# Sweethyh/GaussianImage_plus

Hardware: AMD Instinct MI355X
Metric: training iters/sec (fwd+bwd rasterize) at N Gaussians, 768x512 (higher is better)
Workload: dtype f32; 1 GPU; Cholesky model, N=50000 Gaussians, 768x512, one image per GPU, whole training iterations with the optimizer ON (moving gaussians): tanh/+bound + project fwd + incremental tile binning + rasterize_sum fwd + L2 gradient of the render + rasterize_sum bwd + project bwd + Adam per step; num_points=50000, height=512, width=768, seed=3047

## Files before the change

gaussianimage_plus_amd/csrc/gi2d_common.h:

```cpp
#pragma once
#include <hip/hip_runtime.h>
#include <stdint.h>

#include "gi2d.h"

#define GI2D_WAVE 64
#define GI2D_BLOCK 256

namespace gi2d {

void set_error(const char *msg);
int check_launch(const char *what);

__device__ __forceinline__ int cvt_rzi(float x) {
    if (x != x) return 0;
    x = fminf(fmaxf(x, -2147483648.f), 2147483520.f);
    return (int)x;
}

__device__ __forceinline__ void tile_bbox(float cx, float cy, float pix_radius, int tiles_x,
                                          int tiles_y, int &min_x, int &min_y, int &max_x,
                                          int &max_y) {
#pragma clang fp contract(off)
    const float tcx = cx / (float)GI2D_TILE, tcy = cy / (float)GI2D_TILE;
// ... 55 lines not shown

struct ConicS {
    float ha, hb, hc;
};
__device__ __forceinline__ ConicS scale_conic(float a, float b, float c) {
    const float l2e = 1.4426950408889634f;
    ConicS s;
    s.ha = 0.5f * a * l2e;
    s.hb = b * l2e;
    s.hc = 0.5f * c * l2e;
    return s;
}
__device__ __forceinline__ float row_term_b(const ConicS &s, float dy) { return s.hb * dy; }
__device__ __forceinline__ float row_term_c(const ConicS &s, float dy) { return __builtin_fmaf(s.hc * dy, dy, 0.f); }
__device__ __forceinline__ float pair_sigma(const ConicS &s, float dx, float bdy, float cdy2) {
    return __builtin_fmaf(dx, __builtin_fmaf(s.ha, dx, bdy), cdy2);
}
__device__ __forceinline__ float pair_vis(float sigma_l2) { return __builtin_amdgcn_exp2f(-sigma_l2); }

struct AlphaRule {
    unsigned lim;
    bool clamp;
};
#define GI2D_LIM_ODD 0xffffffffu
__device__ __forceinline__ AlphaRule alpha_rule(float gx, float gy, float a, float b, float c, float opac) {
    AlphaRule r;
    const float s = gx + gy + a + b + c + opac;
    const bool odd = !(__builtin_fabsf(s) <= 3.4028235e38f);
    r.clamp = odd || !(opac <= 1.f);
    const float smax = __builtin_amdgcn_logf(opac * 255.f);
    r.lim = odd ? GI2D_LIM_ODD : (smax >= 0.f ? (unsigned)__float_as_int(smax) + 1u : 0u);
    return r;
}
__device__ __forceinline__ bool pair_lands(float sigma_l2, unsigned lim) { return (unsigned)__float_as_int(sigma_l2) < lim; }
__device__ __forceinline__ bool pair_lands_odd(float sigma_l2, float alpha_unclamped, unsigned lim) {
    unsigned as_written = (!(sigma_l2 < 0.f) & !(fminf(1.f, alpha_unclamped) < (1.f / 255.f))) ? 1u : 0u;
    unsigned fast = pair_lands(sigma_l2, lim) ? 1u : 0u;
    asm volatile("" : "+v"(as_written), "+v"(fast));
    return (lim == GI2D_LIM_ODD ? as_written : fast) != 0u;
}

struct CullBox {
    float x0, x1, y0, y1;
};
#define GI2D_CULL_FULL 3.0e38f
#ifndef GI2D_CULL_MARGIN
#define GI2D_CULL_MARGIN 0.0625f
#endif
__device__ __forceinline__ void cull_extent(float gx, float gy, float a, float b, float c, float opac, float &hx,
                                            float &hy) {
    const float big = GI2D_CULL_FULL;
    hx = hy = big;
    if (!(opac == opac)) return;
    if (!(opac * 255.f >= 1.f)) {
        hx = hy = -1.f;
        return;
    }
    const float det = a * c - b * b;
    if (!(a > 0.f) || !(c > 0.f) || !(det > 0.f)) return;
    const float tau2 = 2.f * __logf(opac * 255.f) * 1.0002f + 1e-3f;
    const float t = tau2 * __builtin_amdgcn_rcpf(det);
    const float ex = __builtin_amdgcn_sqrtf(t * c) * 1.0002f + GI2D_CULL_MARGIN;
    const float ey = __builtin_amdgcn_sqrtf(t * a) * 1.0002f + GI2D_CULL_MARGIN;
    if (!(ex < big) || !(ey < big) || !(gx == gx) || !(gy == gy)) return;
    hx = ex;
    hy = ey;
// ... 24 lines not shown
```

gaussianimage_plus_amd/csrc/gi2d_fast.hip:

```cpp
#include <cstdio>
#include <cstdlib>
#include <cstring>
#include <mutex>
#include <unordered_map>
#include <vector>

#include <hip/hip_ext.h>

#include "gi2d_fused_core.h"
#include "gi2d_batch.h"

namespace gi2d {

__global__ __launch_bounds__(256) void fast_fill_kernel(int n, const float2 *__restrict__ xys,
                                                        const int32_t *__restrict__ radii,
                                                        const float *__restrict__ conics,
                                                        const float *__restrict__ colors,
                                                        const float *__restrict__ opacities, int tiles_x, int tiles_y,
                                                        float radius_clip, PrevBox *__restrict__ prev_box,
                                                        int32_t *__restrict__ lists, RecSets rs,
                                                        int32_t *__restrict__ status) {
    const int g = blockIdx.x * blockDim.x + threadIdx.x;
    begin_binning(g, status);
    const BinRecs recs = recs_for_binning(rs, g == 0);
// ... 25 lines not shown
}

template <int KIND>
__global__ __launch_bounds__(256) void fast_project_fill_kernel(
    int n, float clip_coe, const float2 *__restrict__ means2d, const float *__restrict__ p0,
    const float *__restrict__ p1, float img_w, float img_h, int tiles_x, int tiles_y, float radius_clip,
    float2 *__restrict__ xys, float *__restrict__ depths, int32_t *__restrict__ radii,
    float *__restrict__ conics, int32_t *__restrict__ num_tiles_hit, BinTarget bt) {
    project_fill_one<KIND>(blockIdx.x * blockDim.x + threadIdx.x, n, clip_coe, means2d, p0, p1, img_w, img_h, tiles_x,
                           tiles_y, radius_clip, xys, depths, radii, conics, num_tiles_hit, bt);
}

struct FastFwdLds {
    FwdLds f;
};
static_assert(sizeof(float4) * GI2D_FWD_PAIRBUF >= sizeof(int) * GI2D_FAST_C, "the id buffer of the list head overlays the pair buffers");

template <bool WT>
__global__ __launch_bounds__(256) void fast_fwd_kernel(
    int tiles_x, int tiles_y, int img_w, int img_h, RecSets rs, const float *__restrict__ background,
    int32_t *__restrict__ lists, int2 *__restrict__ tile_bins,
    GaussRec *__restrict__ packed, float4 *__restrict__ partial_g, float4 *__restrict__ partial_big,
    int32_t *__restrict__ status, float *__restrict__ final_Ts, int32_t *__restrict__ final_idx,
    float *__restrict__ out_img) {
    __shared__ FastFwdLds sm;
    __shared__ int grp[32];
    int *ids = reinterpret_cast<int *>(sm.f.pairbuf);
    const int tile = blockIdx.x;
    const int tx = tile % tiles_x, ty = tile / tiles_x;
    const int tid = threadIdx.x;
    const float4 *recs = recs_for_tile_pass(rs, blockIdx.x == 0 && tid == 0);
    if (tid == 0) fwd_stage_dummy(sm.f);
    const float tx0 = (float)(tx * GI2D_TILE), ty0 = (float)(ty * GI2D_TILE);
    const int L = tile_list_head<false>(
        ids, grp, tile, tx, ty, recs, lists, tile_bins, status, [&](int, const BinRec &br) { return br; },
        [&](int rank, int g, const BinRec &br) {
            const GaussRec &r = br.r;
            int slot = partial_slot(g, br.box, tx, ty, br.pool);
            float4 *row = partial_row(slot, partial_g, partial_big, tiles_x * tiles_y * GI2D_TILE_LIST_CAP, status);
            if (!row) slot = GI2D_NO_ROW;
            if (rank < GI2D_TILE_LIST_CAP) {
                const AlphaRule ar = alpha_rule(r.gx, r.gy, r.a, r.b, r.c, r.opac);
                const unsigned mask = cull_word_ext(r.gx, r.gy, br.hx, br.hy, tx0, ty0, img_h, ar.clamp);
                fwd_stage_entry(sm.f, rank, r, mask, ar.lim);
                float4 *dst = reinterpret_cast<float4 *>(packed + (size_t)tile * GI2D_TILE_LIST_CAP + rank);
                store16<WT>(dst, make_float4(r.gx, r.gy, r.a, r.b), packed);
                store16<WT>(dst + 1, make_float4(r.c, r.opac, r.cr, r.cg), packed);
                store16<WT>(dst + 2, make_float4(r.cb, __int_as_float(slot), __int_as_float(g), __int_as_float((int)mask)), packed);
            } else if (row) {
                const float4 z = make_float4(0.f, 0.f, 0.f, 0.f);
                row[0] = z;
                row[1] = z;
                row[2] = z;
            }
        }, Inbox{nullptr}, head_row_load(lists, tile, false));
    __syncthreads();
    const int len = L > GI2D_TILE_LIST_CAP ? GI2D_TILE_LIST_CAP : L;
    const bool nothing = background != nullptr && !tile_pass_has_members(rs);
    if (final_idx)
        fwd_rasterize_staged<true, WT>(sm.f, len, list_base(tile), tx, ty, img_w, img_h, nothing, background,
                                       final_Ts, final_idx, out_img);
    else
        fwd_rasterize_staged<false, WT>(sm.f, len, list_base(tile), tx, ty, img_w, img_h, nothing, background,
                                        final_Ts, final_idx, out_img);
    if (tid == 0 && L > 0) status[0] = 1;
}

__global__ __launch_bounds__(256) void fast_background_kernel(int img_w, int img_h,
                                                              const int32_t *__restrict__ status,
                                                              const float *__restrict__ background,
                                                              float *__restrict__ out_img) {
    if (status[0] > 0) return;
    const size_t npix = (size_t)img_w * img_h;
    for (size_t p = blockIdx.x * (size_t)blockDim.x + threadIdx.x; p < npix; p += (size_t)gridDim.x * blockDim.x) {
        out_img[3 * p] = background[0];
        out_img[3 * p + 1] = background[1];
        out_img[3 * p + 2] = background[2];
    }
}

template <bool WITH_ABS, bool WT>
// ... 224 lines not shown
    BinTarget bt;
    int32_t *tile_order;
};

template <int KIND, bool FILL_NEXT>
__global__ __launch_bounds__(256) void fast_reduce_project_kernel(
    int n, int role_blocks, float2 *xys, int32_t *radii, float *conics, int tiles_x, int tiles_y, float radius_clip,
    PrevBox *prev_box, const int32_t *__restrict__ gids_sorted, const int2 *__restrict__ tile_bins,
    const float4 *__restrict__ partial_g, const float4 *__restrict__ partial_big, const float *__restrict__ p0,
    const float *__restrict__ p1, float img_w, float img_h, float2 *__restrict__ v_xy, float *__restrict__ v_conic,
    float *__restrict__ v_rgb, float *__restrict__ v_opacity, float4 *__restrict__ v_abs_xy,
    float *__restrict__ v_cov2d, float2 *__restrict__ v_mean2d, float *__restrict__ v_p0, float *__restrict__ v_p1,
    NextProject next) {
    int block = blockIdx.x;
    if (FILL_NEXT) {
        if (block >= 2 * role_blocks) {
            compute_tile_order(tile_bins, tiles_x * tiles_y, next.tile_order);
            return;
        }
        if (block >= role_blocks) {
            project_fill_one<KIND>((block - role_blocks) * blockDim.x + threadIdx.x, n, next.clip_coe, next.means2d, p0,
                                   p1, img_w, img_h, tiles_x, tiles_y, radius_clip, xys, next.depths, radii, conics,
                                   next.num_tiles_hit, next.bt);
            return;
        }
    }
    const int g = block * blockDim.x + threadIdx.x;
    int2 box = make_int2(0, 0);
    int pool = -1;
    float conic[3] = {0.f, 0.f, 0.f};
    int radius = 0;
    if (g < n) {
        if (FILL_NEXT) {
            const float4 *rec = recs_of_last_pass(next.bt.recs) + 4 * (size_t)g;
            const float4 q0 = rec[0], q1 = rec[1], q2 = rec[2], q3 = rec[3];
            conic[0] = q0.z, conic[1] = q0.w, conic[2] = q1.x;
            box = make_int2(__float_as_int(q2.w), __float_as_int(q3.x));
            radius = __float_as_int(q3.y);
            pool = __float_as_int(q3.z);
        } else {
            const PrevBox pb = prev_box[g];
            box = make_int2(pb.x, pb.y), pool = pb.z;
            conic[0] = conics[3 * g], conic[1] = conics[3 * g + 1], conic[2] = conics[3 * g + 2];
            radius = radii[g];
        }
    }
    float par[3] = {0.f, 0.f, 0.f};
    if (g < n) {
        if (KIND == kScaleRot)
            par[0] = p0[2 * g], par[1] = p0[2 * g + 1], par[2] = p1[g];
        else if (KIND == kCholesky)
            par[0] = p0[3 * g], par[1] = p0[3 * g + 1], par[2] = p0[3 * g + 2];
    }
    float acc[11];
    reduce_one(g, box, pool, tiles_x * tiles_y * GI2D_TILE_LIST_CAP, partial_g, partial_big, acc);
    if (g >= n) return;
    store_grads(g, acc, v_xy, v_conic, v_rgb, v_opacity, v_abs_xy);
    ProjGrad r;
    r.g11 = r.g12 = r.g22 = r.o0 = r.o1 = r.o2 = 0.f;
    r.v_mean = make_float2(0.f, 0.f);
    if (radius > 0) {
        const float vc[3] = {acc[2], acc[3], acc[4]};
        r = project_bwd_one<KIND>(0, par, par + 2, img_w, img_h, conic, make_float2(acc[0], acc[1]), vc);
    }
    store_proj_grad(g, KIND == kScaleRot, r, v_cov2d, v_mean2d, v_p0, v_p1);
}

static int check_ws(const char *what, void *ws, size_t ws_bytes, int n, int tiles_x, int tiles_y) {
    if (n < 0 || tiles_x < 0 || tiles_y < 0) {
        set_error("fast path: negative size");
        return GI2D_ERR_INVALID_ARGUMENT;
// ... 644 lines not shown
```

gaussianimage_plus_amd/csrc/gi2d_fast_internal.h:

```cpp
#pragma once
#include <atomic>
#include <type_traits>

#include "gi2d_project_core.h"
#include "gi2d_raster_core.h"

namespace gi2d {


#define GI2D_FAST_C 1024
#define GI2D_FAST_HDR 16
#define GI2D_INBOX_WORDS 64
#define GI2D_INBOX_SLOTS (32 * GI2D_INBOX_WORDS)
#define GI2D_INBOX_MAX_TILES 1536
#define GI2D_FAST_LROW (GI2D_FAST_C + GI2D_FAST_HDR + GI2D_INBOX_WORDS)
#define GI2D_FAST_EPT (GI2D_FAST_C / 256)
#define GI2D_FAST_S 32
#ifndef GI2D_FILL_BATCH
#define GI2D_FILL_BATCH 16
#endif
#ifndef GI2D_REDUCE_BATCH
#define GI2D_REDUCE_BATCH 8
#endif
#define GI2D_BIG_TILES_F 32
// ... 58 lines not shown
    GaussRec *packed;
    PrevBox *prev_box;
    float4 *recs;
    int32_t *ver;
    float4 *partial_g;
    float4 *partial_big;
    int32_t *tile_order;
    int32_t *big_tile;
    size_t bytes;
};
static FastWs carve_fast(void *base, int n, int num_tiles) {
    FastWs w;
    char *b = (char *)base;
    size_t off = 0;
    const size_t t = (size_t)(num_tiles > 0 ? num_tiles : 1), nn = (size_t)(n > 0 ? n : 1);
    w.inbox_recs = nullptr;
    w.lists = (int32_t *)(b + off);
    w.gids_sorted = w.lists;
    off += align_up(t * GI2D_FAST_LROW * sizeof(int32_t));
    w.tile_bins = (int32_t *)(b + off);
    off += align_up(t * 2 * sizeof(int32_t));
    w.packed = (GaussRec *)(b + off);
    off += align_up(t * GI2D_TILE_LIST_CAP * sizeof(GaussRec));
    w.tile_order = (int32_t *)(b + off);
    off += align_up(t * sizeof(int32_t));
    w.big_tile = (int32_t *)(b + off);
    off += align_up(t * sizeof(int32_t));
    w.prev_box = (PrevBox *)(b + off);
    off += align_up(nn * sizeof(PrevBox));
    w.ver = (int32_t *)(b + off);
    off += align_up(64 * sizeof(int32_t));
    w.recs = (float4 *)(b + off);
    off += 2 * align_up(nn * 4 * sizeof(float4));
    w.partial_g = (float4 *)(b + off);
    off += align_up(nn * GI2D_FAST_S * GI2D_FAST_ROW * sizeof(float4));
    w.partial_big = (float4 *)(b + off);
    off += align_up(t * GI2D_TILE_LIST_CAP * GI2D_FAST_ROW * sizeof(float4));
    w.bytes = off;
    return w;
}
static inline bool wt_fits(const FastWs &w, int num_tiles, size_t image_bytes) {
    const size_t rows_span = (size_t)((const char *)w.partial_big - (const char *)w.partial_g) +
                             (size_t)(num_tiles > 0 ? num_tiles : 1) * GI2D_TILE_LIST_CAP * GI2D_FAST_ROW * sizeof(float4);
    const size_t packed_span = (size_t)(num_tiles > 0 ? num_tiles : 1) * GI2D_TILE_LIST_CAP * sizeof(GaussRec);
    return rows_span < 0xffff0000ull && packed_span < 0xffff0000ull && image_bytes < 0xffff0000ull;
}
static inline size_t inbox_bytes(long long num_tiles) {
    if (num_tiles < 1 || num_tiles > GI2D_INBOX_MAX_TILES) return 0;
    return align_up((size_t)num_tiles * GI2D_INBOX_SLOTS * 4 * sizeof(float4));
}
__host__ __device__ __forceinline__ int list_base(int tile) { return tile * GI2D_FAST_LROW + GI2D_FAST_HDR; }

__device__ __forceinline__ int2 pack_box(int mnx, int mny, int mxx, int mxy) {
    return make_int2(mnx | (mxx << 16), mny | (mxy << 16));
}
struct FillPending {
    int c[GI2D_FILL_BATCH], p[GI2D_FILL_BATCH];
    int nt, w, mnx, mny, omnx, omxx, omny, omxy, di, dj;
    int pool;
    bool live;
};
#ifdef GI2D_INBOX_STATS
#define GI2D_INBOX_STAT(word) atomicAdd(&lists[word], 1)
#else
#define GI2D_INBOX_STAT(word) \
    do {                      \
// ... 120 lines not shown
template <bool INBOX = false>
__device__ __forceinline__ void fill_diff_end(int g, FillPending &f, int tiles_x, int32_t *__restrict__ lists,
                                              const InboxFill *in = nullptr) {
    if (f.nt == 0) return;
    fill_trip_store(f, g, lists);
    for (int base = GI2D_FILL_BATCH; base < f.nt; base += GI2D_FILL_BATCH) {
        fill_trip_issue<INBOX>(f, base, tiles_x, lists, in);
        fill_trip_store(f, g, lists);
    }
}
__device__ __forceinline__ void fill_diff(int g, bool member, int mnx, int mny, int mxx, int mxy, int tiles_x,
                                          PrevBox old, PrevBox *__restrict__ prev_box, int32_t *__restrict__ lists) {
    FillPending f = fill_diff_begin(g, member, mnx, mny, mxx, mxy, tiles_x, old, prev_box, lists);
    fill_diff_end(g, f, tiles_x, lists);
}
__device__ __forceinline__ bool bin_box(const float2 xy, int rad, float radius_clip, int tiles_x, int tiles_y, int &mnx,
                                        int &mny, int &mxx, int &mxy) {
    mnx = mny = mxx = mxy = 0;
    if (rad <= 0 || (float)rad < radius_clip) return false;
    tile_bbox(xy.x, xy.y, (float)rad, tiles_x, tiles_y, mnx, mny, mxx, mxy);
    return mxx > mnx && mxy > mny;
}
__device__ __forceinline__ bool tile_member(const float2 xy, int rad, float radius_clip, int tiles_x, int tiles_y,
                                            int tx, int ty, int &mnx, int &mny, int &mxx, int &mxy) {
    return bin_box(xy, rad, radius_clip, tiles_x, tiles_y, mnx, mny, mxx, mxy) && tx >= mnx && tx < mxx && ty >= mny &&
           ty < mxy;
}
struct RecSets {
    float4 *base;
    int32_t *ver;
    unsigned stride;
    int seq;
};
#define GI2D_VER_ANY 2
#define GI2D_VER_ANY_SEQ 3
#define GI2D_VER_LATEST 4
#define GI2D_VER_WORDS 5
static_assert(GI2D_VER_WORDS <= 16, "the stamps share the version words' 64 bytes; word 16 onwards has other owners");
struct BinRecs {
    float4 *recs;
    int32_t *any;
    int stamp, seq;
};
__device__ __forceinline__ BinRecs recs_for_binning(const RecSets &rs, bool writer) {
    const int c = rs.ver[0];
    BinRecs b;
    b.recs = rs.base + (size_t)((c + 1) & 1) * rs.stride;
    b.any = rs.ver + GI2D_VER_ANY;
    b.stamp = c + 1;
    b.seq = rs.seq;
    if (writer) rs.ver[1] = c + 1, rs.ver[GI2D_VER_LATEST] = rs.seq;
    return b;
}
__device__ __forceinline__ void note_member(const BinRecs &b) { b.any[0] = b.stamp, b.any[GI2D_VER_ANY_SEQ - GI2D_VER_ANY] = b.seq; }
__device__ __forceinline__ bool tile_pass_has_members(const RecSets &rs) {
    return rs.ver[GI2D_VER_ANY] == rs.ver[1] && rs.ver[GI2D_VER_ANY_SEQ] == rs.ver[GI2D_VER_LATEST];
}
__device__ __forceinline__ const float4 *recs_for_tile_pass(const RecSets &rs, bool writer) {
    const int b = rs.ver[1];
    if (writer) rs.ver[0] = b;
    return rs.base + (size_t)(b & 1) * rs.stride;
}
__device__ __forceinline__ const float4 *recs_of_last_pass(const RecSets &rs) {
    return rs.base + (size_t)(rs.ver[0] & 1) * rs.stride;
}
inline std::atomic<unsigned> g_call_seq{1};
static inline RecSets rec_sets(const FastWs &w, int n) {
    RecSets rs;
    rs.seq = (int)(g_call_seq.fetch_add(1, std::memory_order_relaxed) & 0x7fffffffu);
    rs.base = w.recs;
    rs.stride = (unsigned)(align_up((size_t)(n > 0 ? n : 1) * 4 * sizeof(float4)) / sizeof(float4));
    rs.ver = w.ver;
    return rs;
}
struct BinTarget {
    const float *colors, *opacities;
    PrevBox *prev_box;
    int32_t *lists;
    RecSets recs;
    int32_t *status;
};

__device__ __forceinline__ void begin_binning(int g, int32_t *__restrict__ status) {
    if (g == 0) {
        status[0] = 0;
        status[1] = 0;
        status[3] = 0;
    }
}
__device__ __forceinline__ void make_record(float4 (&q)[4], int g, float2 xy, float a, float b, float c, float opac,
                                            float cr, float cg, float cb, int2 box, int radius, int pool) {
    float hx, hy;
    cull_extent(xy.x, xy.y, a, b, c, opac, hx, hy);
    q[0] = make_float4(xy.x, xy.y, a, b);
    q[1] = make_float4(c, opac, cr, cg);
    q[2] = make_float4(cb, hx, hy, __int_as_float(box.x));
    q[3] = make_float4(__int_as_float(box.y), __int_as_float(radius), __int_as_float(pool), __int_as_float(g));
}
__device__ __forceinline__ void store_record(float4 *__restrict__ recs, int g, const float4 (&q)[4]) {
    float4 *r = recs + 4 * (size_t)g;
    r[0] = q[0], r[1] = q[1], r[2] = q[2], r[3] = q[3];
}
__device__ __forceinline__ void write_record(float4 *__restrict__ recs, int g, float2 xy, float a, float b, float c,
                                             float opac, float cr, float cg, float cb, int2 box, int radius, int pool) {
    float4 q[4];
    make_record(q, g, xy, a, b, c, opac, cr, cg, cb, box, radius, pool);
    store_record(recs, g, q);
}
struct BinRec {
    GaussRec r;
    float hx, hy;
    int2 box;
    int pool;
};
__device__ __forceinline__ BinRec record_of(const float4 q0, const float4 q1, const float4 q2, const float4 q3, int g) {
    BinRec o;
    o.r.gx = q0.x, o.r.gy = q0.y, o.r.a = q0.z, o.r.b = q0.w;
    o.r.c = q1.x, o.r.opac = q1.y, o.r.cr = q1.z, o.r.cg = q1.w;
    o.r.cb = q2.x, o.r.slot = -1, o.r.gid = g, o.r.pad = 0;
    o.hx = q2.y, o.hy = q2.z;
    o.box = make_int2(__float_as_int(q2.w), __float_as_int(q3.x));
    o.pool = __float_as_int(q3.z);
    return o;
}
__device__ __forceinline__ BinRec load_record(const float4 *__restrict__ recs, int g) {
    const float4 *p = recs + 4 * (size_t)g;
    const float4 q0 = p[0], q1 = p[1], q2 = p[2];
    const float4 q3 = p[3];
    return record_of(q0, q1, q2, q3, g);
}
__device__ __forceinline__ BinRec load_inbox_record(const float4 *__restrict__ p) {
    const float4 q0 = p[0], q1 = p[1], q2 = p[2];
    const float4 q3 = p[3];
    return record_of(q0, q1, q2, q3, __float_as_int(q3.w));
}
__device__ __forceinline__ void unpack_box(int2 box, int &mnx, int &mny, int &mxx, int &mxy) {
    mnx = box.x & 0xffff, mxx = (int)((unsigned)box.x >> 16), mny = box.y & 0xffff, mxy = (int)((unsigned)box.y >> 16);
}
template <bool INBOX = false, class Between>
__device__ __forceinline__ void bin_one(int g, float2 xy, int radius, bool has_tiles, float ka, float kb, float kc,
                                        float opac, float cr, float cg, float cb, int tiles_x, int tiles_y,
                                        float radius_clip, PrevBox old_box, PrevBox *__restrict__ prev_box,
                                        int32_t *__restrict__ lists, const BinRecs &br, Between between,
                                        InboxFill *in = nullptr) {
    int mnx, mny, mxx, mxy;
    const bool member = bin_box(xy, radius, radius_clip, tiles_x, tiles_y, mnx, mny, mxx, mxy) && has_tiles;
    {
        const unsigned long long mm = __ballot(member);
        if (mm != 0ull && (int)(threadIdx.x & 63) == __builtin_ctzll(mm)) note_member(br);
    }
    float4 *recs = br.recs;
    const int2 box = member ? pack_box(mnx, mny, mxx, mxy) : make_int2(0, 0);
    if constexpr (INBOX) {
        make_record(in->q, g, xy, ka, kb, kc, opac, cr, cg, cb, box, radius, old_box.z);
        FillPending f = fill_diff_begin<true>(g, member, mnx, mny, mxx, mxy, tiles_x, old_box, prev_box, lists, in);
        in->q[3].z = __int_as_float(f.pool);
        store_record(recs, g, in->q);
        between();
        fill_diff_end<true>(g, f, tiles_x, lists, in);
    } else {
        FillPending f = fill_diff_begin(g, member, mnx, mny, mxx, mxy, tiles_x, old_box, prev_box, lists);
        write_record(recs, g, xy, ka, kb, kc, opac, cr, cg, cb, box, radius, f.pool);
        between();
        fill_diff_end(g, f, tiles_x, lists);
    }
}
__device__ __forceinline__ void bin_one(int g, float2 xy, int radius, bool has_tiles, float ka, float kb, float kc,
                                        float opac, float cr, float cg, float cb, int tiles_x, int tiles_y,
                                        float radius_clip, PrevBox old_box, PrevBox *__restrict__ prev_box,
                                        int32_t *__restrict__ lists, const BinRecs &recs) {
    bin_one(g, xy, radius, has_tiles, ka, kb, kc, opac, cr, cg, cb, tiles_x, tiles_y, radius_clip, old_box, prev_box, lists,
            recs, [] {});
}
template <bool INBOX = false, class Between>
__device__ __forceinline__ void bin_projected(int g, const ProjOut &o, float opac, float cr, float cg, float cb,
                                              int tiles_x, int tiles_y, float radius_clip, PrevBox old_box,
                                              PrevBox *__restrict__ prev_box, int32_t *__restrict__ lists,
                                              const BinRecs &recs, Between between, InboxFill *in = nullptr) {
    bin_one<INBOX>(g, o.xy, o.radius, o.tiles_hit > 0, o.k0, o.k1, o.k2, opac, cr, cg, cb, tiles_x, tiles_y, radius_clip,
                   old_box, prev_box, lists, recs, between, in);
}
__device__ __forceinline__ void bin_projected(int g, const ProjOut &o, float opac, float cr, float cg, float cb,
                                              int tiles_x, int tiles_y, float radius_clip, PrevBox old_box,
                                              PrevBox *__restrict__ prev_box, int32_t *__restrict__ lists,
                                              const BinRecs &recs) {
    bin_projected(g, o, opac, cr, cg, cb, tiles_x, tiles_y, radius_clip, old_box, prev_box, lists, recs, [] {});
}

__device__ __forceinline__ int partial_slot(int g, int2 box, int tx, int ty, int pool) {
    int mnx, mny, mxx, mxy;
    unpack_box(box, mnx, mny, mxx, mxy);
    const int w = mxx - mnx, ntiles = w * (mxy - mny), at = (ty - mny) * w + (tx - mnx);
    if (ntiles <= GI2D_FAST_S) return g * GI2D_FAST_S + at;
    return -(pool + at) - 1;
}
// ... 25 lines not shown
    h.inbox_w = 0u;
    if (inbox) h.inbox_w = (unsigned)row[GI2D_FAST_HDR + GI2D_FAST_C + (threadIdx.x & 63)];
    return h;
}
__device__ __forceinline__ HeadRow head_row_for(const int32_t *__restrict__ lists, const int32_t *__restrict__ order,
                                                int slot, int &tile, bool inbox) {
    HeadRow h = head_row_load(lists, slot, inbox);
    tile = __builtin_amdgcn_readfirstlane(order[slot]);
    if (tile != slot) h = head_row_load(lists, tile, inbox);
    return h;
}
template <bool OPTIMISTIC, int EPT, bool INBOX, class Prep, class Put>
__device__ __forceinline__ int tile_list_head_rows(int *ids, int *grp, int tile, int tx, int ty,
                                                   const float4 *__restrict__ recs, int32_t *__restrict__ row,
                                                   int2 *__restrict__ tile_bins, int32_t *__restrict__ status, Prep prep,
                                                   Put put, int id0, int hdr_count, int hdr_sorted, int count, int sorted,
                                                   unsigned inbox_w, const float4 *__restrict__ inbox) {
    const int tid = threadIdx.x, lane = tid & 63, wv = tid >> 6;
    int my_id[EPT];
    my_id[0] = id0;
    int k_in = 0, ent_id = -1, ent_at = 0;
    unsigned ent_more = 0u;
    decltype(prep(0, BinRec())) st_in;
    const bool any_in = INBOX && __ballot(inbox_w != 0u) != 0ull;
    if (any_in) {
        const int pc = __popc(inbox_w), incl_w = wave_inclusive_scan(pc);
        k_in = wave_read_lane(incl_w, 63);
        const unsigned wd = (unsigned)__shfl((int)inbox_w, tid >> 2, 64);
        const int sh = 8 * (tid & 3);
        const unsigned byte = (wd >> sh) & 0xffu;
        ent_at = count + __shfl(incl_w - pc, tid >> 2, 64) + __popc(wd & ((1u << sh) - 1u));
        if (byte != 0u) {
            const BinRec rin = load_inbox_record(inbox + 4 * (size_t)(tid * 8 + __ffs((int)byte) - 1));
            ent_id = rin.r.gid;
            st_in = prep(ent_id, rin);
            if (ent_at < GI2D_FAST_C) ids[ent_at] = ent_id;
            ent_more = byte & (byte - 1u);
#ifdef GI2D_INBOX_STATS
            atomicAdd(&(row - (size_t)tile * GI2D_FAST_LROW)[5], 1);
            if (ent_more) atomicAdd(&(row - (size_t)tile * GI2D_FAST_LROW)[6], __popc(ent_more));
#endif
            int at = ent_at + 1;
            for (unsigned m = ent_more; m; m &= m - 1u, ++at)
                if (at < GI2D_FAST_C) ids[at] = __float_as_int(inbox[4 * (size_t)(tid * 8 + __ffs((int)m) - 1) + 3].w);
        }
    }
    const int count_all = min(count + k_in, GI2D_FAST_C);
    if (tid == 0 && (hdr_count > GI2D_FAST_C || count + k_in > GI2D_FAST_C)) {
        atomicOr(&status[1], 1);
        atomicOr(&status[2], 1);
    }
    if (tid == 0 && hdr_count + k_in > GI2D_FAST_C / 2) atomicMax(&status[3], hdr_count + k_in);
    if (tid >= count) my_id[0] = -1;
    GI2D_HEAD_TRACE(11);
    BinRec r0;
    bool keep[EPT];
    int pos[EPT];
#pragma unroll
    for (int u = 0; u < EPT; ++u) keep[u] = false, pos[u] = 0;
    if constexpr (EPT > 1) {
#pragma unroll
        for (int u = 1; u < EPT; ++u) my_id[u] = -1;
    }
    const auto member = [&](int2 box) {
        int mnx, mny, mxx, mxy;
        unpack_box(box, mnx, mny, mxx, mxy);
        return tx >= mnx && tx < mxx && ty >= mny && ty < mxy;
    };
    const int rounds = EPT == 1 ? 1 : (count + 255) >> 8;
    const int wv_s = __builtin_amdgcn_readfirstlane(wv);
    decltype(prep(0, BinRec())) st0;
    if ((wv_s << 6) >= count) {
        if (lane == 0) {
#pragma unroll
            for (int u = 0; u < EPT; ++u) grp[wv + 4 * u] = 0, grp[16 + wv + 4 * u] = 0;
        }
    } else {
        if (my_id[0] >= 0) {
            r0 = load_record(recs, my_id[0]);
            keep[0] = member(r0.box);
            if (keep[0]) st0 = prep(my_id[0], r0);
        }
        if constexpr (EPT > 1) {
#pragma unroll
            for (int u = 1; u < EPT; ++u) {
                if (u < rounds) {
                    const int e = tid + 256 * u;
                    if (e < count) {
                        my_id[u] = row[GI2D_FAST_HDR + e];
                        const float4 *p = recs + 4 * (size_t)my_id[u];
                        keep[u] = member(make_int2(__float_as_int(p[2].w), __float_as_int(p[3].x)));
                    }
                }
            }
        }
        GI2D_HEAD_TRACE(12);
#pragma unroll
        for (int u = 0; u < EPT; ++u) {
            if (u < rounds) {
                const int e = tid + 256 * u;
                if (e < count) ids[e] = keep[u] ? my_id[u] : -1;
                const unsigned long long kp = __ballot(keep[u] && e < sorted), ka = __ballot(keep[u] && e >= sorted);
                pos[u] = __popcll(kp & lanemask_lt());
                if (lane == 0) {
                    grp[wv + 4 * u] = __popcll(kp);
                    grp[16 + wv + 4 * u] = __popcll(ka);
                }
            } else if (lane == 0) {
                grp[wv + 4 * u] = 0;
                grp[16 + wv + 4 * u] = 0;
            }
        }
    }
    if (OPTIMISTIC && keep[0] && tid < sorted) put(tid, my_id[0], st0);
    __syncthreads();
    if (any_in && wv == 0 && inbox_w != 0u) row[GI2D_FAST_HDR + GI2D_FAST_C + lane] = 0;
    GI2D_HEAD_TRACE(13);
    const int cnt = (lane < 32 && (lane & 15) < 4 * EPT) ? grp[lane] : 0;
    const int incl = wave_inclusive_scan(cnt);
    const int len = wave_read_lane(incl, 31) + (count_all - count);
    const int wv_u = __builtin_amdgcn_readfirstlane(wv);
    int before[EPT];
#pragma unroll
    for (int u = 0; u < EPT; ++u) before[u] = wave_read_lane(incl - cnt, wv_u + 4 * u);
// ... 250 lines not shown
```

gaussianimage_plus_amd/csrc/gi2d_fused_core.h:

```cpp
#pragma once
#include <cstdint>

#include <hip/hip_runtime.h>

#ifdef GI2D_FUSED_TRACE
namespace gi2d {
__device__ unsigned long long *g_fused_trace = nullptr;
}
#define GI2D_TRACE_AT(wg, i)                                                                        \
    do {                                                                                            \
        if (threadIdx.x == 0 && g_fused_trace) g_fused_trace[(wg) * 16 + (i)] = wall_clock64();     \
    } while (0)
#define GI2D_TRACE(i) GI2D_TRACE_AT(tile, i)
#define GI2D_TRACE_VALUE(i, v)                                                        \
    do {                                                                              \
        if (threadIdx.x == 0 && g_fused_trace) g_fused_trace[tile * 16 + (i)] = (v);  \
    } while (0)
#define GI2D_BWD_TRACE(i) GI2D_TRACE_AT(blockIdx.x, i)
#define GI2D_HEAD_TRACE(i) GI2D_TRACE_AT(tile, i)
#else
#define GI2D_TRACE(i) \
    do {              \
    } while (0)
#define GI2D_TRACE_VALUE(i, v) \
// ... 80 lines not shown
    const int tx = tile % tiles_x, ty = tile / tiles_x;
    const int pool_rows = tiles_x * tiles_y * GI2D_TILE_LIST_CAP;
    static_assert(CAP <= GI2D_TILE_LIST_CAP, "at most the reference's 256 entries of a tile are rasterized");
    const int tid = threadIdx.x, lane = tid & 63, wv = tid >> 6;
    const int lx = fwd_lane_col(tid), ly = tid >> 4;
    const int j = tx * GI2D_TILE + lx, i = ty * GI2D_TILE + ly;
    const bool inside = (i < img_h) && (j < img_w);
    const size_t pix = (size_t)i * img_w + j;

    GI2D_TRACE(0);
    float p0 = 0.f, p1 = 0.f, p2 = 0.f;
    if (inside) {
        p0 = vsrc[3 * pix];
        p1 = vsrc[3 * pix + 1];
        p2 = vsrc[3 * pix + 2];
    }

    if (tid == 0) {
        sm.gA[CAP] = make_float4(0.f, 0.f, 0.f, 0.f);
        sm.gB[CAP] = make_float4(0.f, 0.f, 0.f, 0.f);
        sm.gC[CAP] = make_float2(0.f, 0.f);
    }
    GI2D_TRACE_VALUE(1, (unsigned long long)blockIdx.x);
    const float tx0 = (float)(tx * GI2D_TILE), ty0 = (float)(ty * GI2D_TILE);
    struct Staged {
        float4 A, B;
        float2 C;
        unsigned cull;
        int slot;
    };
    const int L = tile_list_head<true, INBOX>(
        sm.ids, sm.grp, tile, tx, ty, recs, lists, tile_bins, status,
        [&](int g, const BinRec &br) {
            const GaussRec &r = br.r;
            Staged s;
            s.slot = partial_slot(g, br.box, tx, ty, br.pool);
            const ConicS cs = scale_conic(r.a, r.b, r.c);
            s.A = make_float4(r.gx, r.gy, cs.ha, cs.hb);
            s.B = make_float4(cs.hc, r.opac, r.cr, r.cg);
            const AlphaRule ar = alpha_rule(r.gx, r.gy, r.a, r.b, r.c, r.opac);
            s.C = make_float2(r.cb, __int_as_float((int)ar.lim));
            s.cull = cull_word_ext(r.gx, r.gy, br.hx, br.hy, tx0, ty0, img_h, ar.clamp);
            return s;
        },
        [&](int rank, int, const Staged &s) {
            if (rank < CAP) {
                sm.gA[rank] = s.A;
                sm.gB[rank] = s.B;
                sm.gC[rank] = s.C;
                sm.cullw[rank] = s.cull;
                sm.slot[rank] = s.slot;
            } else if (float4 *row = partial_row(s.slot, partial_g, partial_big, pool_rows, status)) {
                const float4 z = make_float4(0.f, 0.f, 0.f, 0.f);
                store16<WT>(row, z, partial_g);
                store16<WT>(row + 1, z, partial_g);
                store16<WT>(row + 2, z, partial_g);
            }
        }, ib, head_row);
    GI2D_TRACE(2);
#if defined(GI2D_STOP_AFTER) && GI2D_STOP_AFTER == 1
    if (L >= 0) return;
#endif
    const int len = L > CAP ? CAP : L;
    GI2D_TRACE(3);

    float *mybuf = reinterpret_cast<float *>(sm.pairbuf) + wv * GI2D_FWD_PAIRBUF;
    float o0, o1, o2;
    int last_unused;
    GI2D_TRACE(4);
    fwd_pixel_half_lists<false, CAP, FWD_UNROLL>(
        sm.lists[wv], mybuf, len, [&](int k) { return sm.cullw[k]; },
        [&](int k) {
            const float4 A = sm.gA[k], B = sm.gB[k];
            FwdRec r;
            r.gx = A.x, r.gy = A.y, r.ha = A.z, r.hb = A.w, r.hc = B.x, r.op = B.y, r.cr = B.z, r.cg = B.w;
// ... 64 lines not shown
```

gaussianimage_plus_amd/csrc/gi2d_raster_core.h:

```cpp
#pragma once
#include "gi2d_common.h"

namespace gi2d {

#define GI2D_ALPHA_MIN (1.f / 255.f)
typedef float v2f __attribute__((ext_vector_type(2)));

struct GaussRec {
    float gx, gy, a, b;
    float c, opac, cr, cg;
    float cb;
    int slot;
    int gid;
    int pad;
};
static_assert(sizeof(GaussRec) == 48, "GaussRec must be 3 x float4");

__device__ __forceinline__ GaussRec load_gaussian(int g, const float2 *__restrict__ xys,
                                                  const float *__restrict__ conics,
                                                  const float *__restrict__ colors,
                                                  const float *__restrict__ opacities) {
    GaussRec r;
    const float2 xy = xys[g];
    r.gx = xy.x;
// ... 207 lines not shown
        const size_t pix = (size_t)i * img_w + j;
        out_img[3 * pix + 0] = o0;
        out_img[3 * pix + 1] = o1;
        out_img[3 * pix + 2] = o2;
    }
}
__device__ __forceinline__ void fwd_store_pixels_wt(float o0, float o1, float o2, int tx, int ty, int img_w,
                                                    float *buf, float *__restrict__ out_img) {
    const int lane = threadIdx.x & 63, wv = threadIdx.x >> 6;
    float *mine = buf + 48 * (lane >> 4) + 3 * fwd_lane_col(lane);
    mine[0] = o0, mine[1] = o1, mine[2] = o2;
    __builtin_amdgcn_wave_barrier();
    if (lane < 48) {
        const int row = lane / 12, piece = lane - 12 * row;
        const float4 v = *reinterpret_cast<const float4 *>(buf + 48 * row + 4 * piece);
        const size_t pix = (size_t)(ty * GI2D_TILE + wv * 4 + row) * img_w + tx * GI2D_TILE;
        store16<true>(reinterpret_cast<float4 *>(out_img + 3 * pix) + piece, v, out_img);
    }
}

struct FwdLds {
    float4 AB[2 * (GI2D_TILE_LIST_CAP + 1)];
    float2 C[GI2D_TILE_LIST_CAP + 2];
    unsigned cullw[GI2D_TILE_LIST_CAP];
    unsigned char lists[4][2 * GI2D_FWD_LISTLEN];
    float4 pairbuf[GI2D_FWD_PAIRBUF_OF(true)];
};

__device__ __forceinline__ void fwd_stage_entry(FwdLds &sm, int k, const GaussRec &r, unsigned cull, unsigned lim) {
    const ConicS s = scale_conic(r.a, r.b, r.c);
    sm.AB[2 * k] = make_float4(r.gx, r.gy, s.ha, s.hb);
    sm.AB[2 * k + 1] = make_float4(s.hc, r.opac, r.cr, r.cg);
    sm.C[k] = make_float2(r.cb, __int_as_float((int)lim));
    sm.cullw[k] = cull;
}
__device__ __forceinline__ void fwd_stage_dummy(FwdLds &sm) {
    sm.AB[2 * GI2D_FWD_DUMMY] = make_float4(0.f, 0.f, 0.f, 0.f);
    sm.AB[2 * GI2D_FWD_DUMMY + 1] = make_float4(0.f, 0.f, 0.f, 0.f);
    sm.C[GI2D_FWD_DUMMY] = make_float2(0.f, 0.f);
}

template <bool NEED_FIDX = true, bool WT = false>
__device__ __forceinline__ void fwd_rasterize_staged(FwdLds &sm, int len, int list_base, int tx, int ty,
                                                     int img_w, int img_h, bool background_fill,
                                                     const float *__restrict__ background,
                                                     float *__restrict__ final_Ts,
                                                     int32_t *__restrict__ final_idx,
                                                     float *__restrict__ out_img) {
    const int tid = threadIdx.x, lane = tid & 63, wv = tid >> 6;
    const int lx = fwd_lane_col(lane), ly = wv * 4 + (lane >> 4);
    const int j = tx * GI2D_TILE + lx, i = ty * GI2D_TILE + ly;
    const bool inside = (i < img_h) && (j < img_w);
    float *mybuf = reinterpret_cast<float *>(sm.pairbuf) + wv * GI2D_FWD_PAIRBUF_OF(NEED_FIDX);
    float o0, o1, o2;
    int last_k;
    fwd_pixel_half_lists<NEED_FIDX>(
        sm.lists[wv], mybuf, len, [&](int k) { return sm.cullw[k]; },
        [&](int k) {
            const float4 A = sm.AB[2 * k], B = sm.AB[2 * k + 1];
            FwdRec r;
            r.gx = A.x, r.gy = A.y, r.ha = A.z, r.hb = A.w, r.hc = B.x, r.op = B.y, r.cr = B.z, r.cg = B.w;
            const float2 c = sm.C[k];
            r.cb = c.x, r.lim = (unsigned)__float_as_int(c.y);
            return r;
        },
        (float)(tx * GI2D_TILE), (float)i, o0, o1, o2, last_k);
// ... 438 lines not shown
```

gaussianimage_plus_amd/csrc/gi2d_train.hip:

```cpp
#include <cstdio>
#include <cstring>
#include <vector>

#include "gi2d_batch.h"
#include "gi2d_quant_core.h"

namespace gi2d {

__device__ __forceinline__ int live_n(const TrainParams &P, int n) { return P.n_dev ? min(n, *P.n_dev) : n; }

struct __attribute__((may_alias)) Row3 {
    float a, b, c;
};
struct __attribute__((may_alias, aligned(8))) Row2 {
    float x, y;
};
__device__ __forceinline__ Row3 load_row3(const float *p, int g) { return *reinterpret_cast<const Row3 *>(p + 3 * (size_t)g); }
__device__ __forceinline__ void store_row3(float *p, int g, float a, float b, float c) {
    Row3 r;
    r.a = a, r.b = b, r.c = c;
    *reinterpret_cast<Row3 *>(p + 3 * (size_t)g) = r;
}
__device__ __forceinline__ float2 load_row2(const float *p, int g) {
    const Row2 r = reinterpret_cast<const Row2 *>(p)[g];
// ... 370 lines not shown
            store_row3(best.feat, g, new_feat.a, new_feat.b, new_feat.c);
            if (best.bound) store_row3(best.bound, g, bound3[0], bound3[1], bound3[2]);
        }
    };
    if (FILL_NEXT) {
        begin_binning(g, next.status);
        const BinRecs recs = recs_for_binning(next.recs, g == 0);
        if constexpr (INBOX) {
            inbox.ib.recs = next.inbox;
            const int old_w = (int)((unsigned)pbox.x >> 16) - (pbox.x & 0xffff), old_h = (int)((unsigned)pbox.y >> 16) - (pbox.y & 0xffff);
            inbox.src.on = old_w > 0 && old_h > 0 && old_w * old_h <= 8;
        }
        asm volatile("" : "+v"(new_xy.x), "+v"(new_xy.y), "+v"(new_chol.a), "+v"(new_chol.b), "+v"(new_chol.c));
        float2 mean2;
        float par2[3];
        activate_rows<KIND>(new_xy, new_chol, bound3, mean2, par2);
        const ProjOut o =
            project_one<KIND>(0, next.clip_coe, &mean2, par2, rot_of<KIND>(par2), img_w, img_h, tiles_x, tiles_y,
                              radius_clip);
#if defined(GI2D_UPDATE_STOP) && GI2D_UPDATE_STOP == 3
        {
            const float all = o.xy.x + o.xy.y + o.k0 + o.k1 + o.k2 + (float)o.radius + (float)o.tiles_hit + rows.mx.x +
                              rows.vx.y + rows.mc.c + rows.vc.a + rows.mf.b + rows.vf.c + new_feat.a + new_feat.b + new_feat.c;
            if (all == 12345.678f) dbg_grads[0] = all;
            return;
        }
#endif
#if defined(GI2D_UPDATE_STOP) && GI2D_UPDATE_STOP == 6
        {
            int mnx, mny, mxx, mxy;
            const bool member = bin_box(o.xy, o.radius, radius_clip, tiles_x, tiles_y, mnx, mny, mxx, mxy) && o.tiles_hit > 0;
            const int2 nw = member ? pack_box(mnx, mny, mxx, mxy) : make_int2(0, 0);
            float4 q[4];
            make_record(q, g, o.xy, o.k0, o.k1, o.k2, opac_next, new_feat.a, new_feat.b, new_feat.c, nw, o.radius, pbox.z);
            float all = (nw.x != pbox.x || nw.y != pbox.y) ? 1.f : 0.f;
#pragma unroll
            for (int k = 0; k < 4; ++k) all += q[k].x + q[k].y + q[k].z + q[k].w;
            all += rows.mx.x + rows.vx.y + rows.mc.c + rows.vc.a + rows.mf.b + rows.vf.c + (float)o.tiles_hit;
            if (all == 12345.678f) dbg_grads[0] = all;
            return;
        }
#endif
        bin_projected<INBOX>(g, o, opac_next, new_feat.a, new_feat.b, new_feat.c, tiles_x, tiles_y, radius_clip, pbox,
                            next.prev_box, next.lists, recs, [&] {
                                if (store_proj) xys[g] = o.xy;
                                radii[g] = o.radius;
                                store_row3(conics, g, o.k0, o.k1, o.k2);
                                if (store_proj) next.num_tiles_hit[g] = o.tiles_hit;
                                store_rest();
                            }, &inbox);
    } else {
        store_rest();
    }
}

template <int KIND, bool FILL_NEXT, bool ADAN, bool INBOX = false>
__global__ __launch_bounds__(256) void train_reduce_update_kernel(UpdateArgs u, AdamStep a_xyz, AdamStep a_chol,
                                                                  AdamStep a_feat, int step, int store_proj) {
    static_assert(FILL_NEXT || !INBOX, "only a binning update kernel has entrants to deliver");
    train_reduce_update_body<KIND, FILL_NEXT, ADAN, INBOX, true>((int)blockIdx.x, blockIdx.x == gridDim.x - 1, u, a_xyz, a_chol,
                                                           a_feat, step, store_proj != 0);
}
template <int KIND, bool FILL_NEXT, bool ADAN>
__global__ __launch_bounds__(256) void train_reduce_update_batched_kernel(const BatchImage *__restrict__ imgs,
                                                                          const int *__restrict__ pg_start,
                                                                          int k_images, AdamStep a_xyz, AdamStep a_chol,
                                                                          AdamStep a_feat, int step, int store_proj) {
// ... 1152 lines not shown
```

Measured before the change: 38030 iters/s.

## Precompute scaled conic and alpha limit in bin records, store raw conic separately

The per-Gaussian binning record now stores the log2-scaled conic terms and the alpha landing limit, computed once in the projection/binning pass. Raw conic values and the radius go into a separate side array. Tile staging in the forward rasterizer then copies the precomputed values instead of recomputing scale_conic and alpha_rule for every tile a Gaussian touches. This costs an extra raw-array write per Gaussian, an extra workspace region, and an extra 16-byte read wherever the raw conic is needed.

```diff
diff --git a/gaussianimage_plus_amd/csrc/gi2d_common.h b/gaussianimage_plus_amd/csrc/gi2d_common.h
--- a/gaussianimage_plus_amd/csrc/gi2d_common.h
+++ b/gaussianimage_plus_amd/csrc/gi2d_common.h
@@ -111,6 +111,7 @@
     r.lim = odd ? GI2D_LIM_ODD : (smax >= 0.f ? (unsigned)__float_as_int(smax) + 1u : 0u);
     return r;
 }
+__device__ __forceinline__ bool alpha_clamp(unsigned lim, float opac) { return lim == GI2D_LIM_ODD || !(opac <= 1.f); }
 __device__ __forceinline__ bool pair_lands(float sigma_l2, unsigned lim) { return (unsigned)__float_as_int(sigma_l2) < lim; }
 __device__ __forceinline__ bool pair_lands_odd(float sigma_l2, float alpha_unclamped, unsigned lim) {
     unsigned as_written = (!(sigma_l2 < 0.f) & !(fminf(1.f, alpha_unclamped) < (1.f / 255.f))) ? 1u : 0u;
diff --git a/gaussianimage_plus_amd/csrc/gi2d_fast.hip b/gaussianimage_plus_amd/csrc/gi2d_fast.hip
--- a/gaussianimage_plus_amd/csrc/gi2d_fast.hip
+++ b/gaussianimage_plus_amd/csrc/gi2d_fast.hip
@@ -81,21 +81,30 @@
     const float4 *recs = recs_for_tile_pass(rs, blockIdx.x == 0 && tid == 0);
     if (tid == 0) fwd_stage_dummy(sm.f);
     const float tx0 = (float)(tx * GI2D_TILE), ty0 = (float)(ty * GI2D_TILE);
+    const float4 *raw = raw_for_tile_pass(rs);
+    struct Entry {
+        BinRec br;
+        float4 raw;
+    };
     const int L = tile_list_head<false>(
-        ids, grp, tile, tx, ty, recs, lists, tile_bins, status, [&](int, const BinRec &br) { return br; },
-        [&](int rank, int g, const BinRec &br) {
-            const GaussRec &r = br.r;
+        ids, grp, tile, tx, ty, recs, lists, tile_bins, status,
+        [&](int g, const BinRec &br) {
+            Entry e;
+            e.br = br, e.raw = raw[g];
+            return e;
+        },
+        [&](int rank, int g, const Entry &e) {
+            const BinRec &br = e.br;
             int slot = partial_slot(g, br.box, tx, ty, br.pool);
             float4 *row = partial_row(slot, partial_g, partial_big, tiles_x * tiles_y * GI2D_TILE_LIST_CAP, status);
             if (!row) slot = GI2D_NO_ROW;
             if (rank < GI2D_TILE_LIST_CAP) {
-                const AlphaRule ar = alpha_rule(r.gx, r.gy, r.a, r.b, r.c, r.opac);
-                const unsigned mask = cull_word_ext(r.gx, r.gy, br.hx, br.hy, tx0, ty0, img_h, ar.clamp);
-                fwd_stage_entry(sm.f, rank, r, mask, ar.lim);
+                const unsigned mask = cull_word_ext(br.A.x, br.A.y, br.hx, br.hy, tx0, ty0, img_h, br.clamp());
+                fwd_stage_staged(sm.f, rank, br.A, br.B, br.C, mask);
                 float4 *dst = reinterpret_cast<float4 *>(packed + (size_t)tile * GI2D_TILE_LIST_CAP + rank);
-                store16<WT>(dst, make_float4(r.gx, r.gy, r.a, r.b), packed);
-                store16<WT>(dst + 1, make_float4(r.c, r.opac, r.cr, r.cg), packed);
-                store16<WT>(dst + 2, make_float4(r.cb, __int_as_float(slot), __int_as_float(g), __int_as_float((int)mask)), packed);
+                store16<WT>(dst, make_float4(br.A.x, br.A.y, e.raw.x, e.raw.y), packed);
+                store16<WT>(dst + 1, make_float4(e.raw.z, br.B.y, br.B.z, br.B.w), packed);
+                store16<WT>(dst + 2, make_float4(br.C.x, __int_as_float(slot), __int_as_float(g), __int_as_float((int)mask)), packed);
             } else if (row) {
                 const float4 z = make_float4(0.f, 0.f, 0.f, 0.f);
                 row[0] = z;
@@ -386,11 +395,11 @@
     int radius = 0;
     if (g < n) {
         if (FILL_NEXT) {
-            const float4 *rec = recs_of_last_pass(next.bt.recs) + 4 * (size_t)g;
-            const float4 q0 = rec[0], q1 = rec[1], q2 = rec[2], q3 = rec[3];
-            conic[0] = q0.z, conic[1] = q0.w, conic[2] = q1.x;
-            box = make_int2(__float_as_int(q2.w), __float_as_int(q3.x));
-            radius = __float_as_int(q3.y);
+            const float4 q3 = recs_of_last_pass(next.bt.recs)[4 * (size_t)g + 3];
+            const float4 rw = raw_of_last_pass(next.bt.recs)[g];
+            conic[0] = rw.x, conic[1] = rw.y, conic[2] = rw.z;
+            box = make_int2(__float_as_int(q3.x), __float_as_int(q3.y));
+            radius = __float_as_int(rw.w);
             pool = __float_as_int(q3.z);
         } else {
             const PrevBox pb = prev_box[g];
diff --git a/gaussianimage_plus_amd/csrc/gi2d_fast_internal.h b/gaussianimage_plus_amd/csrc/gi2d_fast_internal.h
--- a/gaussianimage_plus_amd/csrc/gi2d_fast_internal.h
+++ b/gaussianimage_plus_amd/csrc/gi2d_fast_internal.h
@@ -114,6 +114,7 @@
     off += align_up(64 * sizeof(int32_t));
     w.recs = (float4 *)(b + off);
     off += 2 * align_up(nn * 4 * sizeof(float4));
+    off += align_up(align_up(nn * 4 * sizeof(float4)) / 2);
     w.partial_g = (float4 *)(b + off);
     off += align_up(nn * GI2D_FAST_S * GI2D_FAST_ROW * sizeof(float4));
     w.partial_big = (float4 *)(b + off);
@@ -300,6 +301,9 @@
     unsigned stride;
     int seq;
 };
+__device__ __forceinline__ float4 *raw_of_set(const RecSets &rs, int set) {
+    return rs.base + 2 * (size_t)rs.stride + (size_t)set * (rs.stride >> 2);
+}
 #define GI2D_VER_ANY 2
 #define GI2D_VER_ANY_SEQ 3
 #define GI2D_VER_LATEST 4
@@ -307,6 +311,7 @@
 static_assert(GI2D_VER_WORDS <= 16, "the stamps share the version words' 64 bytes; word 16 onwards has other owners");
 struct BinRecs {
     float4 *recs;
+    float4 *raw;
     int32_t *any;
     int stamp, seq;
 };
@@ -314,6 +319,7 @@
     const int c = rs.ver[0];
     BinRecs b;
     b.recs = rs.base + (size_t)((c + 1) & 1) * rs.stride;
+    b.raw = raw_of_set(rs, (c + 1) & 1);
     b.any = rs.ver + GI2D_VER_ANY;
     b.stamp = c + 1;
     b.seq = rs.seq;
@@ -332,6 +338,8 @@
 __device__ __forceinline__ const float4 *recs_of_last_pass(const RecSets &rs) {
     return rs.base + (size_t)(rs.ver[0] & 1) * rs.stride;
 }
+__device__ __forceinline__ const float4 *raw_for_tile_pass(const RecSets &rs) { return raw_of_set(rs, rs.ver[1] & 1); }
+__device__ __forceinline__ const float4 *raw_of_last_pass(const RecSets &rs) { return raw_of_set(rs, rs.ver[0] & 1); }
 inline std::atomic<unsigned> g_call_seq{1};
 static inline RecSets rec_sets(const FastWs &w, int n) {
     RecSets rs;
@@ -357,38 +365,49 @@
     }
 }
 __device__ __forceinline__ void make_record(float4 (&q)[4], int g, float2 xy, float a, float b, float c, float opac,
-                                            float cr, float cg, float cb, int2 box, int radius, int pool) {
+                                            float cr, float cg, float cb, int2 box, int pool) {
     float hx, hy;
     cull_extent(xy.x, xy.y, a, b, c, opac, hx, hy);
-    q[0] = make_float4(xy.x, xy.y, a, b);
-    q[1] = make_float4(c, opac, cr, cg);
-    q[2] = make_float4(cb, hx, hy, __int_as_float(box.x));
-    q[3] = make_float4(__int_as_float(box.y), __int_as_float(radius), __int_as_float(pool), __int_as_float(g));
+    float gx = xy.x, gy = xy.y, ra = a, rb = b, rc = c, ro = opac;
+    asm volatile("" : "+v"(gx), "+v"(gy), "+v"(ra), "+v"(rb), "+v"(rc), "+v"(ro));
+    const ConicS s = scale_conic(ra, rb, rc);
+    const AlphaRule ar = alpha_rule(gx, gy, ra, rb, rc, ro);
+    q[0] = make_float4(xy.x, xy.y, s.ha, s.hb);
+    q[1] = make_float4(s.hc, opac, cr, cg);
+    q[2] = make_float4(cb, __int_as_float((int)ar.lim), hx, hy);
+    q[3] = make_float4(__int_as_float(box.x), __int_as_float(box.y), __int_as_float(pool), __int_as_float(g));
 }
 __device__ __forceinline__ void store_record(float4 *__restrict__ recs, int g, const float4 (&q)[4]) {
     float4 *r = recs + 4 * (size_t)g;
     r[0] = q[0], r[1] = q[1], r[2] = q[2], r[3] = q[3];
 }
-__device__ __forceinline__ void write_record(float4 *__restrict__ recs, int g, float2 xy, float a, float b, float c,
-                                             float opac, float cr, float cg, float cb, int2 box, int radius, int pool) {
+__device__ __forceinline__ void store_raw(float4 *__restrict__ raw, int g, float a, float b, float c, int radius) {
+    raw[g] = make_float4(a, b, c, __int_as_float(radius));
+}
+__device__ __forceinline__ void write_record(const BinRecs &br, int g, float2 xy, float a, float b, float c, float opac,
+                                             float cr, float cg, float cb, int2 box, int radius, int pool) {
     float4 q[4];
-    make_record(q, g, xy, a, b, c, opac, cr, cg, cb, box, radius, pool);
-    store_record(recs, g, q);
+    make_record(q, g, xy, a, b, c, opac, cr, cg, cb, box, pool);
+    store_record(br.recs, g, q);
+    store_raw(br.raw, g, a, b, c, radius);
 }
 struct BinRec {
-    GaussRec r;
+    float4 A, B;
+    float2 C;
     float hx, hy;
     int2 box;
-    int pool;
+    int pool, gid;
+    __device__ __forceinline__ unsigned lim() const { return (unsigned)__float_as_int(C.y); }
+    __device__ __forceinline__ bool clamp() const { return alpha_clamp(lim(), B.y); }
 };
 __device__ __forceinline__ BinRec record_of(const float4 q0, const float4 q1, const float4 q2, const float4 q3, int g) {
     BinRec o;
-    o.r.gx = q0.x, o.r.gy = q0.y, o.r.a = q0.z, o.r.b = q0.w;
-    o.r.c = q1.x, o.r.opac = q1.y, o.r.cr = q1.z, o.r.cg = q1.w;
-    o.r.cb = q2.x, o.r.slot = -1, o.r.gid = g, o.r.pad = 0;
-    o.hx = q2.y, o.hy = q2.z;
-    o.box = make_int2(__float_as_int(q2.w), __float_as_int(q3.x));
+    o.A = q0, o.B = q1;
+    o.C = make_float2(q2.x, q2.y);
+    o.hx = q2.z, o.hy = q2.w;
+    o.box = make_int2(__float_as_int(q3.x), __float_as_int(q3.y));
     o.pool = __float_as_int(q3.z);
+    o.gid = g;
     return o;
 }
 __device__ __forceinline__ BinRec load_record(const float4 *__restrict__ recs, int g) {
@@ -417,18 +436,18 @@
         const unsigned long long mm = __ballot(member);
         if (mm != 0ull && (int)(threadIdx.x & 63) == __builtin_ctzll(mm)) note_member(br);
     }
-    float4 *recs = br.recs;
     const int2 box = member ? pack_box(mnx, mny, mxx, mxy) : make_int2(0, 0);
     if constexpr (INBOX) {
-        make_record(in->q, g, xy, ka, kb, kc, opac, cr, cg, cb, box, radius, old_box.z);
+        make_record(in->q, g, xy, ka, kb, kc, opac, cr, cg, cb, box, old_box.z);
         FillPending f = fill_diff_begin<true>(g, member, mnx, mny, mxx, mxy, tiles_x, old_box, prev_box, lists, in);
         in->q[3].z = __int_as_float(f.pool);
-        store_record(recs, g, in->q);
+        store_record(br.recs, g, in->q);
+        store_raw(br.raw, g, ka, kb, kc, radius);
         between();
         fill_diff_end<true>(g, f, tiles_x, lists, in);
     } else {
         FillPending f = fill_diff_begin(g, member, mnx, mny, mxx, mxy, tiles_x, old_box, prev_box, lists);
-        write_record(recs, g, xy, ka, kb, kc, opac, cr, cg, cb, box, radius, f.pool);
+        write_record(br, g, xy, ka, kb, kc, opac, cr, cg, cb, box, radius, f.pool);
         between();
         fill_diff_end(g, f, tiles_x, lists);
     }
@@ -520,7 +539,7 @@
         ent_at = count + __shfl(incl_w - pc, tid >> 2, 64) + __popc(wd & ((1u << sh) - 1u));
         if (byte != 0u) {
             const BinRec rin = load_inbox_record(inbox + 4 * (size_t)(tid * 8 + __ffs((int)byte) - 1));
-            ent_id = rin.r.gid;
+            ent_id = rin.gid;
             st_in = prep(ent_id, rin);
             if (ent_at < GI2D_FAST_C) ids[ent_at] = ent_id;
             ent_more = byte & (byte - 1u);
@@ -577,7 +596,7 @@
                     if (e < count) {
                         my_id[u] = row[GI2D_FAST_HDR + e];
                         const float4 *p = recs + 4 * (size_t)my_id[u];
-                        keep[u] = member(make_int2(__float_as_int(p[2].w), __float_as_int(p[3].x)));
+                        keep[u] = member(make_int2(__float_as_int(p[3].x), __float_as_int(p[3].y)));
                     }
                 }
             }
diff --git a/gaussianimage_plus_amd/csrc/gi2d_fused_core.h b/gaussianimage_plus_amd/csrc/gi2d_fused_core.h
--- a/gaussianimage_plus_amd/csrc/gi2d_fused_core.h
+++ b/gaussianimage_plus_amd/csrc/gi2d_fused_core.h
@@ -136,15 +136,10 @@
     const int L = tile_list_head<true, INBOX>(
         sm.ids, sm.grp, tile, tx, ty, recs, lists, tile_bins, status,
         [&](int g, const BinRec &br) {
-            const GaussRec &r = br.r;
             Staged s;
             s.slot = partial_slot(g, br.box, tx, ty, br.pool);
-            const ConicS cs = scale_conic(r.a, r.b, r.c);
-            s.A = make_float4(r.gx, r.gy, cs.ha, cs.hb);
-            s.B = make_float4(cs.hc, r.opac, r.cr, r.cg);
-            const AlphaRule ar = alpha_rule(r.gx, r.gy, r.a, r.b, r.c, r.opac);
-            s.C = make_float2(r.cb, __int_as_float((int)ar.lim));
-            s.cull = cull_word_ext(r.gx, r.gy, br.hx, br.hy, tx0, ty0, img_h, ar.clamp);
+            s.A = br.A, s.B = br.B, s.C = br.C;
+            s.cull = cull_word_ext(br.A.x, br.A.y, br.hx, br.hy, tx0, ty0, img_h, br.clamp());
             return s;
         },
         [&](int rank, int, const Staged &s) {
diff --git a/gaussianimage_plus_amd/csrc/gi2d_raster_core.h b/gaussianimage_plus_amd/csrc/gi2d_raster_core.h
--- a/gaussianimage_plus_amd/csrc/gi2d_raster_core.h
+++ b/gaussianimage_plus_amd/csrc/gi2d_raster_core.h
@@ -263,6 +263,13 @@
     sm.AB[2 * k] = make_float4(r.gx, r.gy, s.ha, s.hb);
     sm.AB[2 * k + 1] = make_float4(s.hc, r.opac, r.cr, r.cg);
     sm.C[k] = make_float2(r.cb, __int_as_float((int)lim));
+    sm.cullw[k] = cull;
+}
+__device__ __forceinline__ void fwd_stage_staged(FwdLds &sm, int k, const float4 A, const float4 B, const float2 C,
+                                                 unsigned cull) {
+    sm.AB[2 * k] = A;
+    sm.AB[2 * k + 1] = B;
+    sm.C[k] = C;
     sm.cullw[k] = cull;
 }
 __device__ __forceinline__ void fwd_stage_dummy(FwdLds &sm) {
diff --git a/gaussianimage_plus_amd/csrc/gi2d_train.hip b/gaussianimage_plus_amd/csrc/gi2d_train.hip
--- a/gaussianimage_plus_amd/csrc/gi2d_train.hip
+++ b/gaussianimage_plus_amd/csrc/gi2d_train.hip
@@ -426,7 +426,7 @@
             const bool member = bin_box(o.xy, o.radius, radius_clip, tiles_x, tiles_y, mnx, mny, mxx, mxy) && o.tiles_hit > 0;
             const int2 nw = member ? pack_box(mnx, mny, mxx, mxy) : make_int2(0, 0);
             float4 q[4];
-            make_record(q, g, o.xy, o.k0, o.k1, o.k2, opac_next, new_feat.a, new_feat.b, new_feat.c, nw, o.radius, pbox.z);
+            make_record(q, g, o.xy, o.k0, o.k1, o.k2, opac_next, new_feat.a, new_feat.b, new_feat.c, nw, pbox.z);
             float all = (nw.x != pbox.x || nw.y != pbox.y) ? 1.f : 0.f;
 #pragma unroll
             for (int k = 0; k < 4; ++k) all += q[k].x + q[k].y + q[k].z + q[k].w;
```

Measured after the change: 37120 iters/s. 2.4% lower.
